# safijari/yag-slam

Measured on AMD Instinct MI355X. Metric: pose hypotheses/sec, higher is better.
Workload: dtype u8

## Files before the change

### yag_slam_amd/csrc/ym_k_region.hpp

```cpp
#pragma once

namespace ym {

#ifndef YM_RG_PROF
#define YM_RG_PROF 0
#endif
#if YM_RG_PROF
#if YM_RG_PROF == 2
#define YM_RG_PH(i) do { if ((i) == 7 || (i) == 8 || (i) == 1 || (i) == 2 || (i) == 5) { const uint32_t t_ = (uint32_t)__builtin_amdgcn_s_memtime(); \
    if ((i) != 5) ph[(i) == 7 ? 0 : (i) == 8 ? 1 : (i) == 1 ? 2 : 3] += t_ - pt; pt = t_; } } while (0)
#else
#define YM_RG_PH(i) do { const uint32_t t_ = (uint32_t)__builtin_amdgcn_s_memtime(); if ((i) >= 2 && (i) <= 5) ph[(i) - 2] += t_ - pt; pt = t_; } while (0)
#endif
#else
#define YM_RG_PH(i) do { } while (0)
#endif

#ifndef YM_RG_ABLATE
#define YM_RG_ABLATE 0
#endif
#ifndef YM_RG_PRIO
#define YM_RG_PRIO 0
#endif
#define YM_RG_W 64
#ifndef YM_RG_H
#define YM_RG_H 80
#endif
#define YM_RG_PITCH 100
#define YM_RG_ROWS (YM_RG_H + 26)
#define YM_RG_SEGS 6
#define YM_RG_CLS (YM_RG_PITCH * YM_RG_ROWS)
#define YM_RG_G 13
#define YM_RG_ZERO (4 * YM_RG_CLS)
#define YM_RG_LDS_BYTES (YM_RG_ZERO + 26 * YM_RG_PITCH + 32)
#define YM_RG_PLANES_SLACK(half_pitch) ((size_t)(2 * YM_RG_ROWS + 2 * YM_RG_H + 2) * (size_t)(half_pitch) + 256)
#define YM_RG_WINDOW_SLACK(pitch) ((size_t)(2 * YM_RG_ROWS + 2 * YM_RG_H + 2) * (size_t)(pitch) + 512)
static_assert(2 * YM_RG_ROWS + 2 * YM_RG_H + 2 >= 2 * (YM_RG_H - 1 + YM_RG_ROWS - 1) + 1 + 1, "YM_RG_PLANES_SLACK does not cover the rows a staged region reads");
static_assert(256 >= 16 * YM_RG_SEGS, "YM_RG_PLANES_SLACK does not cover the bytes a staged row reads");
static_assert(16 * YM_RG_SEGS >= YM_RG_W + 2 * YM_RG_G + 3 && YM_RG_PITCH >= 16 * YM_RG_SEGS && (YM_RG_PITCH / 4) % 2 == 1,
              "a staged row must hold the region, the patch margin and the misalignment, at an odd number of dwords per row");
#define YM_RG_MAX_BINS 8192
#define YM_RG_MAX_REGIONS 96
#define YM_RG_MAX_ENTRIES 28672
#define YM_RG_FLUSH 652
#define YM_BIN_THREADS 1024
#ifndef YM_BIN_MIN_WAVES
#define YM_BIN_MIN_WAVES 8
#endif
#define YM_BIN_LDS_BYTES(nbins, entries, nboxes) ((size_t)(YM_BIN_THREADS / 64 + YM_MAX_COARSE_NT + YM_RG_MAX_BINS / 32 + 1) * 4 + (size_t)(nbins) * 8 + ((size_t)(entries) * 2 + 15) / 16 * 16 + (size_t)(nboxes) * 16)

struct RegionArgs {
    YmGeom g;
    YmLattice lat;
    const uint8_t *grid;
    const uint8_t *planes;
    size_t grid_stride;
    const double2 *ctrig;
    const int32_t *hypcell;
    const YmItemState *states;
    const int32_t *qrep;
    uint16_t *entries;
    size_t entries_stride;
    int32_t *starts;
    size_t starts_stride;
    uint32_t *rbox;
    size_t rbox_stride;
    int32_t nw, parts;
    uint16_t *partial;
    size_t partial_stride;
    int32_t nt_stride, dim_stride;
    int32_t nrx, nry, ng, nbins;
    int32_t force_irregular;
    int32_t fuse_score;
    double *resp;
    size_t sums_stride;
    double *blockmax;
    double *probs;
    size_t probs_stride;
    int32_t n_blocks, pad;
    int32_t rg_h, rg_cls, rg_zero, pad2;
    int32_t rg_w, rg_pitch, nregions, pad3;
    uint32_t *walk;
    int32_t nitems, gpx;
    int32_t rsplit, pad4;
    unsigned long long *stamps;
    int32_t lnw, lparts;
    size_t entries_pstride;
};
__device__ __forceinline__ const int32_t *rg_part_starts(const RegionArgs &a, int qslot, int p) {
    return a.starts + (size_t)qslot * a.starts_stride + (size_t)p * (a.nbins + 1);
}
__device__ __forceinline__ bool rg_part_listed(const RegionArgs &a, int qslot, int p) {
    return a.starts[(size_t)qslot * a.starts_stride + (size_t)a.lparts * (a.nbins + 1) + p] >= 0;
}

__device__ __forceinline__ bool region_entry(const RegionArgs &a, int2 cell, int cx0, int cy0, int k, int &bin, unsigned &entry, int &region,
                                             unsigned &er, unsigned &ex, int bin_nw = -1) {
    const int X = cx0 + cell.x, Y = cy0 + cell.y;
    if (X < 0 || Y < 0) return false;
    const unsigned xc = (unsigned)X >> 1, yc = (unsigned)Y >> 1;
    const unsigned cls = (unsigned)((X & 1) | ((Y & 1) << 1));
#ifdef YM_EXPERIMENTAL
    if (a.rg_w) {
        const unsigned rx = xc / (unsigned)a.rg_w, ry = yc / (unsigned)a.rg_h;
        if ((int)rx >= a.nrx || (int)ry >= a.nry) return false;
        region = (int)((ry * (unsigned)a.nrx + rx) * 4u + cls);
        bin = region * a.lat.nt + k;
        er = yc - ry * (unsigned)a.rg_h;
        ex = xc - rx * (unsigned)a.rg_w;
        entry = er * (unsigned)a.rg_pitch + ex;
        return true;
    }
#endif
    if (yc >= 4096u) return false;
    const unsigned rx = xc / (unsigned)YM_RG_W, ry = __umul24(yc, (unsigned)a.pad2) >> 21;
    if ((int)rx >= a.nrx || (int)ry >= a.nry) return false;
    region = (int)(__umul24(ry, (unsigned)a.nrx) + rx);
    bin = (int)__umul24((unsigned)region, (unsigned)(bin_nw < 0 ? a.lat.nt : bin_nw)) + k;
    er = yc - __umul24(ry, (unsigned)a.rg_h);
    ex = xc - rx * YM_RG_W;
    entry = __umul24(cls, (unsigned)a.rg_cls) + __umul24(er, (unsigned)YM_RG_PITCH) + ex;
    return true;
}

#define YM_BINP_THREADS 512
#define YM_BINP_LDS_BYTES(nbins, entries, nboxes) ((size_t)(YM_BINP_THREADS / 64 + 16 + YM_RG_MAX_BINS / 32 + 1) * 4 + (size_t)(nbins) * 8 + ((size_t)(entries) * 2 + 15) / 16 * 16 + (size_t)(nboxes) * 16)
template <bool YAG, int MAXP>
__global__ __launch_bounds__(YM_BINP_THREADS, MAXP <= 18 ? 4 : 2) void bin_kernel(RegionArgs a) {
    constexpr int NT = YM_BINP_THREADS;
    extern __shared__ __attribute__((aligned(16))) unsigned char bin_smem[];
    int *wave_tot = reinterpret_cast<int *>(bin_smem);
    int *angle_tot = wave_tot + NT / 64;
    unsigned *region_bits = reinterpret_cast<unsigned *>(angle_tot + 16);
    int *regions_used = reinterpret_cast<int *>(region_bits + YM_RG_MAX_BINS / 32);
    unsigned (*cnt)[2] = reinterpret_cast<unsigned (*)[2]>(regions_used + 1);
    unsigned short *ent = reinterpret_cast<unsigned short *>(cnt + a.nbins);
    const int nboxes = a.nregions;
    unsigned (*box)[4] = reinterpret_cast<unsigned (*)[4]>(bin_smem + ((reinterpret_cast<unsigned char *>(ent + a.entries_pstride) - bin_smem) + 15) / 16 * 16);
    const int part = blockIdx.x, qs = blockIdx.y, b = a.qrep[qs], tid = threadIdx.x, lane = tid & 63;
    const YmItemState &st = a.states[b];
    const int nw = a.lnw, k_lo = part * nw, nk = min(a.lat.nt, k_lo + nw) - k_lo;
    const int nq = st.nq;
    const int total = nq * nk;
    const int32_t *cx = a.hypcell + (size_t)b * 2 * a.dim_stride;
    const int cx0 = cx[0], cy0 = cx[a.dim_stride];
    const double off_x = st.off_x, off_y = st.off_y;
    const double2 *ql = reinterpret_cast<const double2 *>(st.ql);
    const double2 *trig = a.ctrig + (size_t)b * a.nt_stride + k_lo;
    int32_t *starts = a.starts + (size_t)qs * a.starts_stride + (size_t)part * (a.nbins + 1);
    int32_t *flag = a.starts + (size_t)qs * a.starts_stride + (size_t)a.lparts * (a.nbins + 1) + part;
    const int pos0 = part * (int)a.entries_pstride;
    double2 *qls = reinterpret_cast<double2 *>(bin_smem + ((reinterpret_cast<unsigned char *>(ent) - bin_smem) + 15) / 16 * 16);
    const bool ql_in_lds = (size_t)(nq + nk) * sizeof(double2) + 16 <= (size_t)a.entries_pstride * 2;
    double2 *trigs = qls + nq;
    if (ql_in_lds) {
        for (int i = tid; i < nq; i += NT) qls[i] = ql[i];
        if (tid < nk) trigs[tid] = trig[tid];
    }
    for (int i = tid; i < a.nbins * 2; i += NT) (&cnt[0][0])[i] = 0u;
    if (tid < 16) angle_tot[tid] = 0;
    if (tid < YM_RG_MAX_BINS / 32) region_bits[tid] = 0u;
    if (tid == 0) *regions_used = 0;
    for (int i = tid; i < nboxes; i += NT) { box[i][0] = 255u; box[i][1] = 0u; box[i][2] = 255u; box[i][3] = 0u; }
    __syncthreads();
    unsigned key[MAXP];
    unsigned rank_hi[(MAXP + 3) / 4];
#pragma unroll
    for (int q = 0; q < (MAXP + 3) / 4; q++) rank_hi[q] = 0u;
    const int per_thread = (total + NT - 1) / NT;
    const int p0 = tid * per_thread;
    int k = p0 / max(nq, 1), i = p0 - k * nq;
    int cur = -1;
    unsigned r0 = 255u, r1 = 0u, x0 = 255u, x1 = 0u;
    auto send_box = [&]() {
        if (cur >= 0) {
            unsigned *bx = box[cur];
            atomicMin(&bx[0], r0); atomicMax(&bx[1], r1); atomicMin(&bx[2], x0); atomicMax(&bx[3], x1);
        }
    };
    bool overflow = per_thread > MAXP;
    auto pass1 = [&](auto point_of, auto trig_of) {
#pragma unroll
        for (int q = 0; q < MAXP; q++) {
            const int pp = p0 + q;
            key[q] = 0xffffffffu;
            if (q < per_thread && pp < total) {
                const double2 cs = trig_of(k);
                const double2 pt = point_of(i);
                int bin, region; unsigned e, er, ex;
                const int2 lc = YAG ? lookup_cell_sem(a.g, pt, cs.x, cs.y, off_x, off_y, st.ylat[0], st.ylat[1]) : lookup_cell(pt, cs.x, cs.y, off_x, off_y, a.g.scale);
                if (region_entry(a, lc, cx0, cy0, k, bin, e, region, er, ex, nw)) {
                    const unsigned rank = (atomicAdd(&cnt[bin][(e >> 1) & 1u], 1u << (16 * (e & 1u))) >> (16 * (e & 1u))) & 0xffffu;
                    key[q] = (rank & 7u) << 29 | (unsigned)bin << 16 | e;
                    rank_hi[q >> 2] |= ((rank >> 3) & 0xffu) << (8 * (q & 3));
                    if (region != cur) { send_box(); cur = region; r0 = r1 = er; x0 = x1 = ex; }
                    else { r0 = min(r0, er); r1 = max(r1, er); x0 = min(x0, ex); x1 = max(x1, ex); }
                }
            }
            if (++i >= nq) { i = 0; k++; }
        }
    };
    if (ql_in_lds) pass1([&](int i_) { return qls[i_]; }, [&](int k_) { return trigs[k_]; });
    else pass1([&](int i_) { return ql[i_]; }, [&](int k_) { return trig[k_]; });
    send_box();
    __syncthreads();
    {
        uint32_t *rb = a.rbox + (size_t)qs * a.rbox_stride;
        for (int r = tid; r < nboxes; r += NT) rb[(size_t)r * a.lparts + part] = box[r][0] | box[r][1] << 8 | box[r][2] << 16 | box[r][3] << 24;
    }
    const int per = (a.nbins + NT - 1) / NT;
    const int first = tid * per;
    int padded_total;
    {
        int local = 0;
        for (int j = 0; j < per; j++)
            if (first + j < a.nbins) {
                const unsigned c01 = cnt[first + j][0], c23 = cnt[first + j][1];
                const int c[4] = {(int)(c01 & 0xffffu), (int)(c01 >> 16), (int)(c23 & 0xffffu), (int)(c23 >> 16)};
                const int padded = (((c[0] + 1) & ~1) + ((c[1] + 1) & ~1) + ((c[2] + 1) & ~1) + ((c[3] + 1) & ~1) + 3) & ~3;
                local += padded;
                if (padded) {
                    atomicAdd(&angle_tot[(first + j) % nw], padded);
                    const int R = (first + j) / nw;
                    atomicOr(&region_bits[R >> 5], 1u << (R & 31));
                }
            }
        int incl = local;
#pragma unroll
        for (int d = 1; d < 64; d <<= 1) {
            const int v = __shfl_up(incl, d);
            if (lane >= d) incl += v;
        }
        if (lane == 63) wave_tot[tid >> 6] = incl;
        __syncthreads();
        if (tid < YM_RG_MAX_BINS / 32 && region_bits[tid]) atomicAdd(regions_used, __popc(region_bits[tid]));
        __syncthreads();
        int base = 0, all = 0;
        for (int w = 0; w < NT / 64; w++) {
            if (w < (tid >> 6)) base += wave_tot[w];
            all += wave_tot[w];
        }
        padded_total = all;
        bool fits = all <= (int)a.entries_pstride && pos0 + all <= 65532 && a.force_irregular != 2 && !overflow;
        for (int kk = 0; kk < nk; kk++) fits = fits && angle_tot[kk] <= a.ng * YM_RG_FLUSH;
        fits = fits && *regions_used <= YM_RG_MAX_REGIONS;
        int run = base + incl - local;
        for (int j = 0; j < per; j++)
            if (first + j < a.nbins) {
                const unsigned c01 = cnt[first + j][0], c23 = cnt[first + j][1];
                const int c[4] = {(int)(c01 & 0xffffu), (int)(c01 >> 16), (int)(c23 & 0xffffu), (int)(c23 >> 16)};
                starts[first + j] = pos0 + run;
                int pos = run;
                unsigned fill[4];
                for (int r = 0; r < 4; r++) {
                    fill[r] = (unsigned)pos;
                    if (fits && (c[r] & 1)) ent[pos + c[r]] = (unsigned short)(a.rg_zero + r);
                    pos += (c[r] + 1) & ~1;
                }
                if (fits && ((pos - run) & 3)) { ent[pos] = (unsigned short)a.rg_zero; ent[pos + 1] = (unsigned short)a.rg_zero; }
                pos = run + ((pos - run + 3) & ~3);
                cnt[first + j][0] = fill[0] | fill[1] << 16;
                cnt[first + j][1] = fill[2] | fill[3] << 16;
                run = pos;
            }
        if (tid == 0) {
            starts[a.nbins] = pos0 + all;
            *flag = fits ? all : -1;
            if (a.stamps && qs == 0 && part == 0) a.stamps[26] = (unsigned long long)all;
        }
        if (!fits) return;
    }
    __syncthreads();
#pragma unroll
    for (int q = 0; q < MAXP; q++) {
        if (key[q] == 0xffffffffu) continue;
        const unsigned bin = (key[q] >> 16) & 0x1fffu, e = key[q] & 0xffffu;
        const unsigned rank = key[q] >> 29 | ((rank_hi[q >> 2] >> (8 * (q & 3))) & 0xffu) << 3;
        const unsigned f = cnt[bin][(e >> 1) & 1u];
        ent[((e & 1u) ? f >> 16 : f & 0xffffu) + rank] = (unsigned short)e;
    }
    __syncthreads();
    uint32_t *out = reinterpret_cast<uint32_t *>(a.entries + (size_t)qs * a.entries_stride + pos0);
    const uint32_t *src = reinterpret_cast<const uint32_t *>(ent);
    for (int i2 = tid; i2 < (padded_total + 1) / 2; i2 += NT) out[i2] = src[i2];
}

typedef unsigned int rg_u32x2 __attribute__((ext_vector_type(2)));
__device__ __forceinline__ void rg_perm_pair(const rg_u32x2 &pa, const rg_u32x2 &qa, const rg_u32x2 &pb, const rg_u32x2 &qb, uint32_t rr,
                                             uint32_t (&e)[4], uint32_t (&o)[4]) {
    const uint32_t s0 = pa.x + pb.x, s1 = pa.y + pb.y, s2 = qa.x + qb.x, s3 = qa.y + qb.y;
    const uint32_t selE = rr * 0x00010001u + 0x0c020c00u, selO = selE + 0x00010001u;
    e[0] = __builtin_amdgcn_perm(s1, s0, selE); o[0] = __builtin_amdgcn_perm(s1, s0, selO);
    e[1] = __builtin_amdgcn_perm(s2, s1, selE); o[1] = __builtin_amdgcn_perm(s2, s1, selO);
    e[2] = __builtin_amdgcn_perm(s3, s2, selE); o[2] = __builtin_amdgcn_perm(s3, s2, selO);
    e[3] = __builtin_amdgcn_perm(0u, s3, selE);
    o[3] = 0u;
}
__device__ __forceinline__ void rg_gather4(uint32_t (&acc)[8], uint32_t lane_off, uint2 ee ) {
    const uint32_t ad0 = lane_off + (ee.x & 0xffffu), ad1 = lane_off + (ee.x >> 16), ad2 = lane_off + (ee.y & 0xffffu), ad3 = lane_off + (ee.y >> 16);
#if YM_RG_ABLATE & 1
    acc[0] += ad0 ^ ad1 ^ ad2 ^ ad3;
    return;
#endif
    rg_u32x2 p0, q0, p1, q1, p2, q2, p3, q3;
    asm volatile("ds_read2_b32 %0, %8 offset1:1\n\tds_read2_b32 %1, %8 offset0:2 offset1:3\n\t"
                 "ds_read2_b32 %2, %9 offset1:1\n\tds_read2_b32 %3, %9 offset0:2 offset1:3\n\t"
                 "ds_read2_b32 %4, %10 offset1:1\n\tds_read2_b32 %5, %10 offset0:2 offset1:3\n\t"
                 "ds_read2_b32 %6, %11 offset1:1\n\tds_read2_b32 %7, %11 offset0:2 offset1:3\n\t"
                 "s_waitcnt lgkmcnt(4)"
                 : "=&v"(p0), "=&v"(q0), "=&v"(p1), "=&v"(q1), "=&v"(p2), "=&v"(q2), "=&v"(p3), "=&v"(q3)
                 : "v"(ad0 & ~3u), "v"(ad1 & ~3u), "v"(ad2 & ~3u), "v"(ad3 & ~3u)
                 : "memory");
    uint32_t e[2][4], o[2][4];
    rg_perm_pair(p0, q0, p1, q1, ad0 & 3u, e[0], o[0]);
    asm volatile("s_waitcnt lgkmcnt(0)" : "+v"(p2), "+v"(q2), "+v"(p3), "+v"(q3) : : "memory");
    rg_perm_pair(p2, q2, p3, q3, ad2 & 3u, e[1], o[1]);
#pragma unroll
    for (int j = 0; j < 4; j++) {
        acc[2 * j] = acc[2 * j] + e[0][j] + e[1][j];
        if (j < 3) acc[2 * j + 1] = acc[2 * j + 1] + o[0][j] + o[1][j];
    }
}

__device__ __forceinline__ void rg_odd(uint32_t (&)[8]) {}

template <int NW, bool WIN = false>
__global__ __launch_bounds__(64 * NW, NW <= 8 ? (3 * NW + 3) / 4 : 1 ) void correlate_region_kernel(RegionArgs a) {
    constexpr int NT = 64 * NW;
    constexpr int PER = (YM_RG_ROWS + (NT / 4) / YM_RG_SEGS - 1) / ((NT / 4) / YM_RG_SEGS);
    __shared__ __attribute__((aligned(16))) unsigned char region[YM_RG_LDS_BYTES];
    __shared__ int rlist[YM_RG_MAX_REGIONS];
    __shared__ uint32_t rboxl[YM_RG_MAX_REGIONS];
    __shared__ unsigned short seginfo[NW][YM_RG_MAX_REGIONS][2];
    __shared__ int rcount;
    int p;
    const int b = xcd_item_of_block_2d(p);
    const int rsplit = a.rsplit > 1 ? a.rsplit : 1, rsi = p / a.parts;
    p -= rsi * a.parts;
    const int tid = threadIdx.x, lane = tid & 63, wave = __builtin_amdgcn_readfirstlane(tid >> 6);
    const YmItemState &st = a.states[b];
    const int nt = a.lat.nt, nx = a.lat.nx, ny = a.lat.ny, ng = a.ng;
    const int k = p * NW + wave;
    const bool kvalid = k < nt;
    const int row = lane & 31, half = lane >> 5;
    const bool job = row < ny && half * YM_RG_G < nx;
    const int half_pitch = a.g.pitch / 2;
    const int plane_bytes = half_pitch * a.g.win_w;
    const uint8_t *__restrict__ planes = a.planes + (size_t)b * a.grid_stride;
    const int32_t *__restrict__ starts = rg_part_starts(a, st.qslot, p);
    const uint16_t *__restrict__ entries = a.entries + (size_t)st.qslot * a.entries_stride;
    const uint32_t lds0 = (uint32_t)(size_t)region;
    const uint32_t lane_off = lds0 + (uint32_t)((job ? row : 0) * YM_RG_PITCH + (half * YM_RG_G < nx ? half * YM_RG_G : 0));
    uint32_t acc[8];
#pragma unroll
    for (int j = 0; j < 8; j++) acc[j] = 0u;
    int in_set = 0, flushed = 0;
    auto flush = [&]() {
        if (flushed < ng) {
            rg_odd(acc);
            store_partial16(a.partial + (size_t)b * a.partial_stride + (((size_t)(rsi * ng + flushed) * nt + k) * 64 + lane) * 16, acc);
        }
#pragma unroll
        for (int j = 0; j < 8; j++) acc[j] = 0u;
        flushed++;
        in_set = 0;
    };
#if !YM_RG_PROF
    YM_STAMP(a, 8);
#endif
#if YM_RG_PROF
    uint32_t ph[4] = {0u, 0u, 0u, 0u};
    uint32_t pt = (uint32_t)__builtin_amdgcn_s_memtime();
    const uint32_t pt_begin = pt;
    const unsigned long long rt_begin = __builtin_amdgcn_s_memrealtime();
#endif
    const bool regular = st.regular[0] && a.force_irregular != 1 && rg_part_listed(a, st.qslot, p);
    if (regular) {
        const int k_lo = p * NW, k_hi = min(nt, k_lo + NW);
        const int nreg = a.nrx * a.nry;
        for (int i = tid; i < (YM_RG_LDS_BYTES - YM_RG_ZERO) / 4; i += NT) reinterpret_cast<uint32_t *>(region + YM_RG_ZERO)[i] = 0u;
        if (wave == 0) {
            int n = 0;
            for (int R0 = 0; R0 < nreg; R0 += 64) {
                const int R = R0 + lane;
                const bool has = R < nreg && starts[(size_t)R * NW] != starts[(size_t)R * NW + (k_hi - k_lo)];
                const unsigned long long mask = __ballot(has);
                const int at = n + __popcll(mask & ((1ull << lane) - 1ull));
                if (has && at % rsplit == rsi) rlist[at / rsplit] = R;
                n += __popcll(mask);
            }
            if (lane == 0) rcount = n > rsi ? (n - rsi + rsplit - 1) / rsplit : 0;
        }
        __syncthreads();
        const int nlist = rcount;
        {
            const uint32_t *rb = a.rbox + (size_t)st.qslot * a.rbox_stride;
            const uint32_t reach = (uint32_t)(nx > YM_RG_G ? 15 + YM_RG_G : 15);
            for (int i = tid; i < nlist; i += NT) {
                const uint32_t v = rb[(size_t)rlist[i] * a.parts + p];
                const uint32_t r0 = v & 0xffu, r1 = min((uint32_t)(YM_RG_ROWS - 1), ((v >> 8) & 0xffu) + (uint32_t)ny - 1u);
                const uint32_t s0 = ((v >> 16) & 0xfcu) >> 4, s1 = min((uint32_t)(YM_RG_SEGS - 1), ((v >> 24) + reach) >> 4);
                rboxl[i] = r0 | r1 << 8 | s0 << 16 | s1 << 24;
            }
        }
        if (kvalid)
            for (int i = lane; i < nlist; i += 64) {
                const int32_t *srow = starts + (size_t)rlist[i] * NW + wave;
                seginfo[wave][i][0] = (unsigned short)srow[0]; seginfo[wave][i][1] = (unsigned short)srow[1];
            }
        __syncthreads();
        constexpr int TPC = WIN ? NT / 2 : NT / 4;
        constexpr int NSEG = WIN ? 2 * YM_RG_SEGS : YM_RG_SEGS;
        constexpr int LPS = TPC / NSEG;
        constexpr int RSTEP = LPS;
        static_assert(LPS >= 1 && LPS * PER >= YM_RG_ROWS, "the copy tasks must cover a class image");
        const uint32_t cls = WIN ? 2u * ((uint32_t)tid / TPC) : (uint32_t)tid / TPC, j = (uint32_t)tid % TPC;
        const uint32_t seg = j % NSEG, r0 = j / NSEG;
        const bool copier = j < (uint32_t)(LPS * NSEG);
        const uint32_t src0 = WIN ? (2u * r0 + (cls >> 1)) * (uint32_t)a.g.pitch + 16u * seg
                                  : (cls & 1u) * (uint32_t)plane_bytes + (2u * r0 + (cls >> 1)) * (uint32_t)half_pitch + 16u * seg;
        const uint32_t src_step = WIN ? 2u * RSTEP * (uint32_t)a.g.pitch : 2u * RSTEP * (uint32_t)half_pitch;
        const uint32_t dst0 = (cls * YM_RG_ROWS + r0) * YM_RG_PITCH + (WIN ? 8u : 16u) * seg;
        uint4 v[PER];
        auto in_box = [&](int q, uint32_t bx, bool seg_in) {
            (void)q; (void)bx;
            return seg_in;
        };
        auto band_in = [&](int q, uint32_t bx) {
            return (uint32_t)(q * RSTEP) <= ((bx >> 8) & 0xffu) && (uint32_t)(q * RSTEP + RSTEP - 1) >= (bx & 0xffu);
        };
        const uint8_t *__restrict__ window = a.grid + (size_t)b * a.grid_stride;
        auto seg_inside = [&](uint32_t bx) {
            return WIN ? copier && seg >= 2u * ((bx >> 16) & 0xffu) && seg <= 2u * (bx >> 24) + 1u
                       : copier && seg >= ((bx >> 16) & 0xffu) && seg <= (bx >> 24);
        };
        auto stage_load = [&](int R, uint32_t bx) {
            const int RX = R % a.nrx, RY = R / a.nrx;
            const uint8_t *src = WIN ? window + ((size_t)(2 * RY * YM_RG_H) * a.g.pitch + (size_t)RX * (2 * YM_RG_W))
                                     : planes + ((size_t)(2 * RY * YM_RG_H) * half_pitch + (size_t)RX * YM_RG_W);
            const bool seg_in = seg_inside(bx);
#pragma unroll
            for (int q = 0; q < PER; q++)
#if YM_RG_ABLATE & 2
                v[q] = make_uint4((uint32_t)(size_t)src, seg_in, bx, q);
#else
                if (band_in(q, bx)) v[q] = *reinterpret_cast<const uint4 *>(src + (in_box(q, bx, seg_in) ? src0 + (uint32_t)q * src_step : 0u));
#endif
        };
        auto stage_store = [&](uint32_t bx) {
            const bool seg_in = seg_inside(bx);
#pragma unroll
            for (int q = 0; q < PER; q++) {
                uint32_t *d = reinterpret_cast<uint32_t *>(region + dst0 + (uint32_t)(q * RSTEP * YM_RG_PITCH));
                if (band_in(q, bx) && in_box(q, bx, seg_in) && (!(YM_RG_ABLATE & 4) || v[q].x == 0x12345u)) {
                    if (WIN) {
                        d[0] = __builtin_amdgcn_perm(v[q].y, v[q].x, 0x06040200u); d[1] = __builtin_amdgcn_perm(v[q].w, v[q].z, 0x06040200u);
                        d[YM_RG_CLS / 4] = __builtin_amdgcn_perm(v[q].y, v[q].x, 0x07050301u); d[YM_RG_CLS / 4 + 1] = __builtin_amdgcn_perm(v[q].w, v[q].z, 0x07050301u);
                    } else { d[0] = v[q].x; d[1] = v[q].y; d[2] = v[q].z; d[3] = v[q].w; }
                }
            }
        };
        auto segment = [&](int ri, int &t0, int &t2) {
            t0 = t2 = 0;
            if (kvalid) {
                t0 = __builtin_amdgcn_readfirstlane((int)seginfo[wave][ri][0]);
                t2 = __builtin_amdgcn_readfirstlane((int)seginfo[wave][ri][1]);
            }
        };
        const uint2 *__restrict__ entries4 = reinterpret_cast<const uint2 *>(entries);
        uint2 ev = make_uint2(0u, 0u), cev = make_uint2(0u, 0u);
        auto entries_load = [&](int t0, int t2) {
            ev = make_uint2(0u, 0u);
            if (t0 + 4 * lane < t2) ev = entries4[(t0 >> 2) + lane];
        };
        auto gather = [&](int lo, int hi) {
            const int lds_hi = min(hi, lo + 256);
#if YM_RG_PRIO
            {
                const int n = hi - lo;
                if (n >= 3 * YM_RG_PRIO) __builtin_amdgcn_s_setprio(3);
                else if (n >= 2 * YM_RG_PRIO) __builtin_amdgcn_s_setprio(2);
                else if (n >= YM_RG_PRIO) __builtin_amdgcn_s_setprio(1);
            }
#endif
            if (lo < lds_hi) {
                const int n4 = (lds_hi - lo) >> 2;
                for (int c = 0; c < n4; c++) {
                    rg_gather4(acc, lane_off, make_uint2(__builtin_amdgcn_readlane(cev.x, c), __builtin_amdgcn_readlane(cev.y, c)));
                    in_set += 4;
                    if (in_set == YM_RG_FLUSH) flush();
                }
            }
            for (int c = lds_hi; c < hi; c += 4) {
                rg_gather4(acc, lane_off, entries4[c >> 2]);
                in_set += 4;
                if (in_set == YM_RG_FLUSH) flush();
            }
#if YM_RG_PRIO
            __builtin_amdgcn_s_setprio(0);
#endif
        };
        int s0 = 0, s2 = 0;
        if (nlist > 0) {
            const uint32_t bx = __builtin_amdgcn_readfirstlane(rboxl[0]);
            segment(0, s0, s2);
            entries_load(s0, s2);
            stage_load(rlist[0], bx);
            stage_store(bx);
            cev = ev;
        }
        __syncthreads();
        YM_RG_PH(0);
        for (int ri = 0; ri < nlist; ri++) {
            const bool has_next = ri + 1 < nlist;
            int n0 = 0, n2 = 0;
            uint32_t nbx = 0u;
            if (has_next) {
                nbx = __builtin_amdgcn_readfirstlane(rboxl[ri + 1]);
                segment(ri + 1, n0, n2);
                YM_RG_PH(7);
                entries_load(n0, n2);
                YM_RG_PH(8);
                stage_load(rlist[ri + 1], nbx);
            }
            YM_RG_PH(1);
            gather(s0, s2);
            YM_RG_PH(2);
            __syncthreads();
            YM_RG_PH(3);
            if (has_next) {
                stage_store(nbx);
                cev = ev;
            }
            s0 = n0; s2 = n2;
            YM_RG_PH(4);
            __syncthreads();
            YM_RG_PH(5);
        }
    } else if (kvalid && job && rsi == 0) {
        const uint8_t *__restrict__ grid = a.grid + (size_t)b * a.grid_stride;
        const unsigned limit = (unsigned)(a.g.pitch * a.g.win_w);
        const int32_t *cx = a.hypcell + (size_t)b * 2 * a.dim_stride;
        const int32_t *cy = cx + a.dim_stride;
        const double2 cs = a.ctrig[(size_t)b * a.nt_stride + k];
        const double2 *ql = reinterpret_cast<const double2 *>(st.ql);
        const int nq = st.nq;
        const double add_x = a.g.semantics == 1 ? st.ylat[0] : st.off_x, add_y = a.g.semantics == 1 ? st.ylat[1] : st.off_y;
        for (int g = 0; g < ng; g++) {
            for (int j = 0; j < YM_RG_G; j++) {
                const int ix = half * YM_RG_G + j;
                if (ix >= nx) break;
                const int base = cy[row] * lin_pitch(a.g) + cx[ix];
                unsigned sum = 0;
                const int i1 = min(nq, (g + 1) * YM_RG_FLUSH);
                for (int i = g * YM_RG_FLUSH; i < i1; i++)
                    sum += cell_value(a.g, grid, limit, (unsigned)(base + lookup_offset_sem(a.g, ql[i], cs.x, cs.y, st.off_x, st.off_y, add_x, add_y, lin_pitch(a.g))));
                acc[2 * (j >> 2) + (j & 1)] += sum << (16 * ((j >> 1) & 1));
            }
            flush();
        }
    }
#if !YM_RG_PROF
    YM_STAMP(a, 9);
#endif
#if YM_RG_PROF
    auto prof_out = [&]() {
        if (a.stamps && lane == 0) {
            for (int i = 0; i < 4; i++) atomicAdd(a.stamps + 10 + i, (unsigned long long)ph[i]);
            atomicAdd(a.stamps + 8, (unsigned long long)(pt - pt_begin));
            atomicAdd(a.stamps + 9, __builtin_amdgcn_s_memrealtime() - rt_begin);
        }
    };
#endif
    if (!a.fuse_score) {
        if (!kvalid) return;
        while (flushed < ng) flush();
        return;
    }
    unsigned long long *pmax = reinterpret_cast<unsigned long long *>(region);
    const int nxy = nx * ny;
    double *dpen = reinterpret_cast<double *>(region) + ((nxy + 1) & ~1);
    __syncthreads();
    for (int i = tid; i < nxy; i += NT) {
        pmax[i] = 0ull;
        const int iy = i / nx, ix = i - iy * nx;
        const double x = -a.lat.off_x + ix * a.lat.step_x, y = -a.lat.off_y + iy * a.lat.step_y;
        dpen[i] = dist_penalty(a.g, x * x + y * y);
    }
    __syncthreads();
    if (kvalid) {
        unsigned tot[YM_RG_G];
        rg_odd(acc);
#pragma unroll
        for (int j = 0; j < YM_RG_G; j++) tot[j] = (acc[2 * (j >> 2) + (j & 1)] >> (16 * ((j >> 1) & 1))) & 0xffffu;
        for (int f = 0; f < min(flushed, ng); f++) {
            const uint16_t *pp = a.partial + (size_t)b * a.partial_stride + (((size_t)f * nt + k) * 64 + lane) * 16;
#pragma unroll
            for (int j = 0; j < YM_RG_G; j++) tot[j] += pp[j];
        }
        const double ct = st.center[2];
        const int nq = st.nq;
        const double angle = (ct - a.lat.angle_off) + k * a.lat.angle_res;
        const int ncb = (nxy + YM_SCORE_THREADS - 1) / YM_SCORE_THREADS;
        double bmax0 = -1.0, bmax1 = -1.0;
        const int c0 = row * nx + half * YM_RG_G, cb0 = job ? c0 / YM_SCORE_THREADS : 0;
#pragma unroll
        for (int j = 0; j < YM_RG_G; j++) {
            const int ix = half * YM_RG_G + j;
            if (job && ix < nx) {
                const int c = row * nx + ix;
                const double r = hyp_response_dp(a.g, a.lat.penalize, tot[j], nq, dpen[c], angle, ct);
                a.resp[(size_t)b * a.sums_stride + (size_t)k * nxy + c] = r;
                if (c / YM_SCORE_THREADS == cb0) bmax0 = r > bmax0 ? r : bmax0;
                else bmax1 = r > bmax1 ? r : bmax1;
                if (r > 0.0) atomicMax(&pmax[c], (unsigned long long)__double_as_longlong(r));
            }
        }
        for (int cb = 0; cb < ncb; cb++) {
            const double mine = !job ? -1.0 : cb == cb0 ? bmax0 : cb == cb0 + 1 ? bmax1 : -1.0;
            const double m = wave_reduce(mine, OpMaxD());
            if (lane == 0) a.blockmax[(size_t)b * a.n_blocks + (size_t)k * ncb + cb] = m;
        }
    }
    __syncthreads();
    for (int i = tid; i < nxy; i += NT)
        if (pmax[i]) atomicMax(reinterpret_cast<unsigned long long *>(a.probs) + (size_t)b * a.probs_stride + i, pmax[i]);
#if YM_RG_PROF
    YM_RG_PH(6);
    prof_out();
#endif
}


}
```

Measured before the change: 13.55 billion.

## Streamline bin_kernel pass1 with branchless bounds, LDS-address keys and segment iteration

Rewrites the binning pass so each point's validity is checked by two unsigned compares against precomputed x/y limits. Region fields now come from shifts and masks instead of divisions. The per-point key stores the raw LDS counter address plus rank, with entry values packed two per register, which removes the bin/rank decode and the counter reload in the scatter pass. The query/angle walk is restructured into segments with the trig hoisted per angle, and the region/angle index in the prefix loop is tracked incrementally instead of using modulo and division. It relies on address-space casts and bit-field assumptions (YM_RG_W==64, rank fitting in 11 bits), which adds fragility.

Result: no change. 13.67 billion, median of 6 (+0.9%).

```diff
diff --git a/yag_slam_amd/csrc/ym_k_region.hpp b/yag_slam_amd/csrc/ym_k_region.hpp
--- a/yag_slam_amd/csrc/ym_k_region.hpp
+++ b/yag_slam_amd/csrc/ym_k_region.hpp
@@ -94,14 +94,29 @@
     return a.starts[(size_t)qslot * a.starts_stride + (size_t)a.lparts * (a.nbins + 1) + p] >= 0;
 }
 
+__device__ __forceinline__ int rg_round_int(double v) { return (int)copysign(fabs(v) + 0.5, v); }
+static_assert(YM_RG_W == 64, "region_fields takes the column region and the byte inside it as bit fields of the window column");
+__device__ __forceinline__ unsigned region_xlim(const RegionArgs &a) { return (unsigned)max(a.nrx, 0) * (2u * YM_RG_W); }
+__device__ __forceinline__ unsigned region_ylim(const RegionArgs &a) { return min(8192u, (unsigned)max(a.nry, 0) * 2u * (unsigned)a.rg_h); }
+__device__ __forceinline__ void region_fields(const RegionArgs &a, int X, int Y, int k, int bin_nw, int &bin, unsigned &entry, int &region,
+                                              unsigned &er, unsigned &ex) {
+    const unsigned yc = ((unsigned)Y >> 1) & 0xfffu, rx = (unsigned)X >> 7;
+    const unsigned ry = (unsigned)__umul24(yc, (unsigned)a.pad2 & 0x3fffffu) >> 21;
+    region = (int)(__umul24(ry, (unsigned)a.nrx) + rx);
+    bin = (int)__umul24((unsigned)region, (unsigned)bin_nw) + k;
+    er = yc - __umul24(ry, (unsigned)a.rg_h);
+    ex = ((unsigned)X >> 1) & (unsigned)(YM_RG_W - 1);
+    const unsigned cls = (unsigned)((X & 1) | ((Y & 1) << 1));
+    entry = __umul24(cls, (unsigned)a.rg_cls) + __umul24(er, (unsigned)YM_RG_PITCH) + ex;
+}
 __device__ __forceinline__ bool region_entry(const RegionArgs &a, int2 cell, int cx0, int cy0, int k, int &bin, unsigned &entry, int &region,
                                              unsigned &er, unsigned &ex, int bin_nw = -1) {
     const int X = cx0 + cell.x, Y = cy0 + cell.y;
-    if (X < 0 || Y < 0) return false;
-    const unsigned xc = (unsigned)X >> 1, yc = (unsigned)Y >> 1;
-    const unsigned cls = (unsigned)((X & 1) | ((Y & 1) << 1));
 #ifdef YM_EXPERIMENTAL
     if (a.rg_w) {
+        if (X < 0 || Y < 0) return false;
+        const unsigned xc = (unsigned)X >> 1, yc = (unsigned)Y >> 1;
+        const unsigned cls = (unsigned)((X & 1) | ((Y & 1) << 1));
         const unsigned rx = xc / (unsigned)a.rg_w, ry = yc / (unsigned)a.rg_h;
         if ((int)rx >= a.nrx || (int)ry >= a.nry) return false;
         region = (int)((ry * (unsigned)a.nrx + rx) * 4u + cls);
@@ -112,14 +127,8 @@
         return true;
     }
 #endif
-    if (yc >= 4096u) return false;
-    const unsigned rx = xc / (unsigned)YM_RG_W, ry = __umul24(yc, (unsigned)a.pad2) >> 21;
-    if ((int)rx >= a.nrx || (int)ry >= a.nry) return false;
-    region = (int)(__umul24(ry, (unsigned)a.nrx) + rx);
-    bin = (int)__umul24((unsigned)region, (unsigned)(bin_nw < 0 ? a.lat.nt : bin_nw)) + k;
-    er = yc - __umul24(ry, (unsigned)a.rg_h);
-    ex = xc - rx * YM_RG_W;
-    entry = __umul24(cls, (unsigned)a.rg_cls) + __umul24(er, (unsigned)YM_RG_PITCH) + ex;
+    if (!((int)((unsigned)X < region_xlim(a)) & (int)((unsigned)Y < region_ylim(a)))) return false;
+    region_fields(a, X, Y, k, bin_nw < 0 ? a.lat.nt : bin_nw, bin, entry, region, er, ex);
     return true;
 }
 
@@ -145,8 +154,11 @@
     const int32_t *cx = a.hypcell + (size_t)b * 2 * a.dim_stride;
     const int cx0 = cx[0], cy0 = cx[a.dim_stride];
     const double off_x = st.off_x, off_y = st.off_y;
-    const double2 *ql = reinterpret_cast<const double2 *>(st.ql);
-    const double2 *trig = a.ctrig + (size_t)b * a.nt_stride + k_lo;
+    typedef double rg_f64x2 __attribute__((ext_vector_type(2)));
+    typedef const __attribute__((address_space(1))) rg_f64x2 *gptr;
+    const gptr ql = (gptr) reinterpret_cast<const rg_f64x2 *>(st.ql);
+    const gptr trig = (gptr) reinterpret_cast<const rg_f64x2 *>(a.ctrig + (size_t)b * a.nt_stride + k_lo);
+    auto table = [](gptr t, int i) { const rg_f64x2 v = t[i]; return make_double2(v.x, v.y); };
     int32_t *starts = a.starts + (size_t)qs * a.starts_stride + (size_t)part * (a.nbins + 1);
     int32_t *flag = a.starts + (size_t)qs * a.starts_stride + (size_t)a.lparts * (a.nbins + 1) + part;
     const int pos0 = part * (int)a.entries_pstride;
@@ -154,8 +166,8 @@
     const bool ql_in_lds = (size_t)(nq + nk) * sizeof(double2) + 16 <= (size_t)a.entries_pstride * 2;
     double2 *trigs = qls + nq;
     if (ql_in_lds) {
-        for (int i = tid; i < nq; i += NT) qls[i] = ql[i];
-        if (tid < nk) trigs[tid] = trig[tid];
+        for (int i = tid; i < nq; i += NT) qls[i] = table(ql, i);
+        if (tid < nk) trigs[tid] = table(trig, tid);
     }
     for (int i = tid; i < a.nbins * 2; i += NT) (&cnt[0][0])[i] = 0u;
     if (tid < 16) angle_tot[tid] = 0;
@@ -163,65 +175,87 @@
     if (tid == 0) *regions_used = 0;
     for (int i = tid; i < nboxes; i += NT) { box[i][0] = 255u; box[i][1] = 0u; box[i][2] = 255u; box[i][3] = 0u; }
     __syncthreads();
-    unsigned key[MAXP];
-    unsigned rank_hi[(MAXP + 3) / 4];
-#pragma unroll
-    for (int q = 0; q < (MAXP + 3) / 4; q++) rank_hi[q] = 0u;
+    unsigned key[MAXP], ekey[(MAXP + 1) / 2];
+#pragma unroll
+    for (int q = 0; q < MAXP; q++) key[q] = 0xffffffffu;
+#pragma unroll
+    for (int q = 0; q < (MAXP + 1) / 2; q++) ekey[q] = 0u;
     const int per_thread = (total + NT - 1) / NT;
     const int p0 = tid * per_thread;
-    int k = p0 / max(nq, 1), i = p0 - k * nq;
-    int cur = -1;
+    const int nval = min(max(total - p0, 0), per_thread);
+    int k = p0 / max(nq, 1), i0 = p0 - k * nq;
+    if (nval == 0) k = i0 = 0;
+    int nxt = min(nq - i0, nval);
+    typedef __attribute__((address_space(3))) unsigned lds_u32;
+    typedef __attribute__((address_space(3))) unsigned short lds_u16;
+    const unsigned cnt_at = (unsigned)(size_t)(__attribute__((address_space(3))) unsigned char *)reinterpret_cast<unsigned char *>(cnt);
+    unsigned xlim = region_xlim(a), ylim = region_ylim(a);
+    asm("" : "+s"(ylim));
+    int cur = 0;
     unsigned r0 = 255u, r1 = 0u, x0 = 255u, x1 = 0u;
     auto send_box = [&]() {
-        if (cur >= 0) {
-            unsigned *bx = box[cur];
-            atomicMin(&bx[0], r0); atomicMax(&bx[1], r1); atomicMin(&bx[2], x0); atomicMax(&bx[3], x1);
-        }
+        unsigned *bx = box[cur];
+        atomicMin(&bx[0], r0); atomicMax(&bx[1], r1); atomicMin(&bx[2], x0); atomicMax(&bx[3], x1);
     };
     bool overflow = per_thread > MAXP;
-    auto pass1 = [&](auto point_of, auto trig_of) {
+    auto pass1 = [&](auto point_of, auto next_segment, auto trig_of) {
+        double2 cs = trig_of(k);
 #pragma unroll
         for (int q = 0; q < MAXP; q++) {
-            const int pp = p0 + q;
-            key[q] = 0xffffffffu;
-            if (q < per_thread && pp < total) {
-                const double2 cs = trig_of(k);
-                const double2 pt = point_of(i);
+            if (q >= per_thread) continue;
+            if (q == nxt) {
+                if (q == nval) { xlim = 0u; nxt = -1; }
+                else { k++; cs = trig_of(k); next_segment(); nxt = min(nxt + nq, nval); }
+            }
+            const double2 pt = point_of(q);
+            int2 lc;
+            if (YAG) lc = lookup_cell_sem(a.g, pt, cs.x, cs.y, off_x, off_y, st.ylat[0], st.ylat[1]);
+            else {
+                const double ox = cs.x * pt.x - cs.y * pt.y;
+                const double oy = cs.y * pt.x + cs.x * pt.y;
+                lc = make_int2(rg_round_int(((ox + off_x) - off_x) * a.g.scale), rg_round_int(((oy + off_y) - off_y) * a.g.scale));
+            }
+            const int X = cx0 + lc.x, Y = cy0 + lc.y;
+            if ((int)((unsigned)X < xlim) & (int)((unsigned)Y < ylim)) {
                 int bin, region; unsigned e, er, ex;
-                const int2 lc = YAG ? lookup_cell_sem(a.g, pt, cs.x, cs.y, off_x, off_y, st.ylat[0], st.ylat[1]) : lookup_cell(pt, cs.x, cs.y, off_x, off_y, a.g.scale);
-                if (region_entry(a, lc, cx0, cy0, k, bin, e, region, er, ex, nw)) {
-                    const unsigned rank = (atomicAdd(&cnt[bin][(e >> 1) & 1u], 1u << (16 * (e & 1u))) >> (16 * (e & 1u))) & 0xffffu;
-                    key[q] = (rank & 7u) << 29 | (unsigned)bin << 16 | e;
-                    rank_hi[q >> 2] |= ((rank >> 3) & 0xffu) << (8 * (q & 3));
-                    if (region != cur) { send_box(); cur = region; r0 = r1 = er; x0 = x1 = ex; }
-                    else { r0 = min(r0, er); r1 = max(r1, er); x0 = min(x0, ex); x1 = max(x1, ex); }
-                }
-            }
-            if (++i >= nq) { i = 0; k++; }
+                region_fields(a, X, Y, k, nw, bin, e, region, er, ex);
+                const unsigned at = cnt_at + ((unsigned)bin << 3) + ((unsigned)X & 6u), sh = (at << 3) & 16u;
+                const unsigned got = __hip_atomic_fetch_add((lds_u32 *)(size_t)(at & ~2u), 1u << sh, __ATOMIC_RELAXED, __HIP_MEMORY_SCOPE_WORKGROUP);
+                key[q] = (got >> sh) << 21 | at;
+                ekey[q >> 1] = (q & 1) ? __builtin_amdgcn_perm(e, ekey[q >> 1], 0x05040100u) : e;
+                if (region != cur) { send_box(); cur = region; r0 = 255u; r1 = 0u; x0 = 255u; x1 = 0u; }
+                r0 = min(r0, er); r1 = max(r1, er); x0 = min(x0, ex); x1 = max(x1, ex);
+            }
         }
     };
-    if (ql_in_lds) pass1([&](int i_) { return qls[i_]; }, [&](int k_) { return trigs[k_]; });
-    else pass1([&](int i_) { return ql[i_]; }, [&](int k_) { return trig[k_]; });
-    send_box();
+    if (ql_in_lds) {
+        const double2 *seg = qls + i0;
+        pass1([&](int q) { return seg[q]; }, [&]() { seg -= nq; }, [&](int k_) { return trigs[k_]; });
+    } else {
+        int seg = i0;
+        pass1([&](int q) { return table(ql, min(max(seg + q, 0), nq - 1)); }, [&]() { seg -= nq; }, [&](int k_) { return table(trig, min(k_, nk - 1)); });
+    }
+    if (nboxes > 0) send_box();
     __syncthreads();
     {
-        uint32_t *rb = a.rbox + (size_t)qs * a.rbox_stride;
-        for (int r = tid; r < nboxes; r += NT) rb[(size_t)r * a.lparts + part] = box[r][0] | box[r][1] << 8 | box[r][2] << 16 | box[r][3] << 24;
+        uint32_t *rb = a.rbox + (size_t)qs * a.rbox_stride + part;
+#pragma unroll 1
+        for (int r = tid; r < nboxes; r += NT) rb[(unsigned)r * (unsigned)a.lparts] = box[r][0] | box[r][1] << 8 | box[r][2] << 16 | box[r][3] << 24;
     }
     const int per = (a.nbins + NT - 1) / NT;
     const int first = tid * per;
     int padded_total;
     {
         int local = 0;
-        for (int j = 0; j < per; j++)
+        int R = first / nw, ka = first - R * nw;
+        for (int j = 0; j < per; j++, ka = ka + 1 == nw ? 0 : ka + 1, R += ka == 0)
             if (first + j < a.nbins) {
                 const unsigned c01 = cnt[first + j][0], c23 = cnt[first + j][1];
                 const int c[4] = {(int)(c01 & 0xffffu), (int)(c01 >> 16), (int)(c23 & 0xffffu), (int)(c23 >> 16)};
                 const int padded = (((c[0] + 1) & ~1) + ((c[1] + 1) & ~1) + ((c[2] + 1) & ~1) + ((c[3] + 1) & ~1) + 3) & ~3;
                 local += padded;
                 if (padded) {
-                    atomicAdd(&angle_tot[(first + j) % nw], padded);
-                    const int R = (first + j) / nw;
+                    atomicAdd(&angle_tot[ka], padded);
                     atomicOr(&region_bits[R >> 5], 1u << (R & 31));
                 }
             }
@@ -273,11 +307,9 @@
     __syncthreads();
 #pragma unroll
     for (int q = 0; q < MAXP; q++) {
-        if (key[q] == 0xffffffffu) continue;
-        const unsigned bin = (key[q] >> 16) & 0x1fffu, e = key[q] & 0xffffu;
-        const unsigned rank = key[q] >> 29 | ((rank_hi[q >> 2] >> (8 * (q & 3))) & 0xffu) << 3;
-        const unsigned f = cnt[bin][(e >> 1) & 1u];
-        ent[((e & 1u) ? f >> 16 : f & 0xffffu) + rank] = (unsigned short)e;
+        if (q >= per_thread || key[q] == 0xffffffffu) continue;
+        const unsigned f = *(const lds_u16 *)(size_t)(key[q] & 0x1fffffu);
+        ent[f + (key[q] >> 21)] = (unsigned short)((q & 1) ? ekey[q >> 1] >> 16 : ekey[q >> 1]);
     }
     __syncthreads();
     uint32_t *out = reinterpret_cast<uint32_t *>(a.entries + (size_t)qs * a.entries_stride + pos0);
```
